# PabloAlvarado/gpitch

Measured on AMD Instinct MI355X. Metric: ELBO-steps/sec, higher is better.
Workload: dtype f64

## Files before the change

gpitch_amd/_lib.py:

```python
import ctypes as C
import os

import numpy as np

_HERE = os.path.dirname(os.path.abspath(__file__))
LIB_PATH = os.environ.get("GPITCH_AMD_LIB") or os.path.join(_HERE, "libgpitch_hip.so")

GP_OK, GP_ERR_BAD_ARG, GP_ERR_NOT_PD, GP_ERR_HIP, GP_ERR_NO_DEVICE, GP_ERR_WORKSPACE, GP_ERR_UNSUPPORTED = range(7)

(KERN_MATERN12, KERN_MATERN32, KERN_MATERN52, KERN_RBF, KERN_MERCER_MATERN12SM, KERN_MATERN12SM, KERN_MATERN32SM,
 KERN_MERCER_MATERN52SM) = range(8)
NLIN_LOGISTIC, NLIN_SOFTPLUS, NLIN_GAUSS = range(3)
(TIMER_KUF_BUILD, TIMER_COND_A, TIMER_COND_LTA, TIMER_NT_GEMM, TIMER_KUF_BAR, TIMER_CHOL, TIMER_LIK, TIMER_SMALL_GEMM,
 TIMER_HYPER, TIMER_KUF_BUILD_SM) = range(10)
TIMER_NAMES = ["kuf_build", "cond_A", "cond_LTA", "nt_gemm", "kuf_bar", "chol", "lik", "small_gemm", "hyper",
               "kuf_build_sm"]

ABI_SYMBOLS = [
    "gp_create", "gp_destroy", "gp_sync", "gp_last_error", "gp_abi_version", "gp_debug_wave_takes", "gp_debug_gemm",
    "gp_debug_hyper_contract", "gp_debug_hyper_records", "gp_debug_hyper_lean_takes", "gp_debug_cov_build", "gp_last_not_pd_index",
    "gp_kernel_build", "gp_kernel_build_f32", "gp_kernel_diag", "gp_chol_workspace_bytes", "gp_kuu_cholesky", "gp_cholesky_inplace",
    "gp_conditional_workspace_bytes", "gp_conditional_diag", "gp_conditional_diag_f32", "gp_conditional_diag_f32w", "gp_conditional_full_workspace_bytes", "gp_conditional_full", "gp_gauss_kl_workspace_bytes", "gp_gauss_kl", "gp_gauss_kl_matrix", "gp_mpd_varexp",
    "gp_mpd_predict_moments", "gp_pdgp_predict_moments", "gp_pdgp_predict_moments_reuse",
    "gp_pdgp_create", "gp_pdgp_destroy", "gp_pdgp_num_params", "gp_pdgp_layout", "gp_pdgp_workspace_bytes",
    "gp_pdgp_set_workspace", "gp_pdgp_set_precision", "gp_pdgp_set_gp_precision", "gp_pdgp_set_grad_needs", "gp_pdgp_set_overlap", "gp_pdgp_set_frames_ascending", "gp_pdgp_set_qform", "gp_pdgp_far_field", "gp_pdgp_far_field_backward", "gp_debug_pdgp_far_ranges", "gp_pdgp_set_far_act", "gp_pdgp_far_field_act", "gp_pdgp_set_scan_far", "gp_pdgp_scan_far", "gp_pdgp_set_h_far", "gp_pdgp_h_far", "gp_debug_pdgp_act_ranges", "gp_pdgp_elbo", "gp_pdgp_elbo_begin", "gp_pdgp_elbo_end", "gp_pdgp_create_subset", "gp_pdgp_cond_begin", "gp_pdgp_cond_end", "gp_pdgp_predict", "gp_pdgp_predict_reuse",
    "gp_pdgp_sample", "gp_pdgp_sample_reuse", "gp_pdgp_sample_workspace_bytes",
    "gp_overlap_merge", "gp_transform_register_logistic", "gp_transform_forward", "gp_transform_backward", "gp_poll_not_pd", "gp_check_not_pd", "gp_take_not_pd", "gp_adam_step",
    "gp_pdgp_natgrad_workspace_bytes", "gp_pdgp_natgrad_step",
    "gp_pdgp_natgrad_adaptive_workspace_bytes", "gp_pdgp_natgrad_step_adaptive", "gp_pdgp_natgrad_counts",
    "gp_sgpr_create", "gp_sgpr_destroy", "gp_sgpr_num_params", "gp_sgpr_workspace_bytes", "gp_sgpr_set_workspace", "gp_sgpr_set_precision",
    "gp_sgpr_bound", "gp_sgpr_bound_grad", "gp_sgpr_residual_grad", "gp_sgpr_exchange_doubles", "gp_sgpr_bound_begin", "gp_sgpr_bound_end", "gp_sgpr_set_graphs", "gp_sgpr_eval_counts", "gp_sgpr_predict_f", "gp_sgpr_predict_f_full", "gp_sgpr_predict_source_full", "gp_sgpr_predict_source_workspace_bytes", "gp_sgpr_predict_source", "gp_sgpr_predict_source_sparse",
    "gp_sgpr_sample_source_sparse", "gp_sgpr_sample_source_workspace_bytes",
    "gp_sgpr_predict_source_ssm", "gp_sgprb_predict_source_ssm", "gp_ssm_smooth_workspace_bytes",
    "gp_sgpr_exact_loglik_grad", "gp_sgprb_exact_loglik_grad", "gp_ssm_score_workspace_bytes",
    "gp_sgpr_sample_source_ssm", "gp_sgprb_sample_source_ssm", "gp_ssm_sample_workspace_bytes",
    "gp_sgprb_create", "gp_sgprb_destroy", "gp_sgprb_num_params", "gp_sgprb_num_windows", "gp_sgprb_workspace_bytes",
    "gp_sgprb_set_workspace", "gp_sgprb_bound_grad", "gp_sgprb_set_graphs", "gp_sgprb_eval_counts",
    "gp_sgprb_set_inducing_counts",
    "gp_sgprb_predict_f", "gp_sgprb_predict_source_workspace_bytes", "gp_sgprb_predict_source", "gp_sgprb_predict_source_sparse", "gp_sgprb_sample_source_sparse",
    "gp_timers_enable", "gp_timers_reset", "gp_timers_read",
    "gp_comm_unique_id", "gp_comm_create", "gp_comm_destroy", "gp_comm_world", "gp_comm_rank", "gp_comm_allreduce_sum",
    "gp_pdgp_elbo_pitch_sharded", "gp_pdgp_elbo_gp_sharded", "gp_sgpr_bound_grad_sharded",
    "gp_segment_gram_workspace_bytes", "gp_segment_gram", "gp_autocorr", "gp_kernfit_eval",
# ... 105 lines not shown
    if _lib is not None:
        return _lib
    import torch
    if not os.path.exists(LIB_PATH):
        raise ImportError("gpitch_amd: %s not found — build it with `python -c 'import __graft_entry__ as g; "
                          "g.build()'` (hipcc --offload-arch=gfx950); there is no CPU fallback" % LIB_PATH)
    lib = C.CDLL(LIB_PATH)
    vp, i32, i64, dbl, sz = C.c_void_p, C.c_int32, C.c_int64, C.c_double, C.c_size_t
    KD = C.POINTER(KernelDesc)
    sig = {
        "gp_create": (i32, [i32, vp, C.POINTER(vp)]),
        "gp_destroy": (i32, [vp]),
        "gp_sync": (i32, [vp]),
        "gp_last_error": (C.c_char_p, [vp]),
        "gp_abi_version": (i32, []),
        "gp_debug_wave_takes": (i32, [i32, i32, i32, i32]),
        "gp_debug_gemm": (i32, [vp, C.POINTER(DebugGemmProblem), i32, i32, i32, C.POINTER(DebugGemmFlags), i32, i32, i32, vp, sz,
                                C.POINTER(i32)]),
        "gp_debug_hyper_contract": (i32, [vp, i32, C.POINTER(DebugHyperItem), C.POINTER(DebugHyperFinish), i32,
                                          C.POINTER(DebugHyperFlags), vp, sz, C.POINTER(i32), C.POINTER(i32)]),
        "gp_debug_hyper_records": (i64, [i32, i32]),
        "gp_debug_hyper_lean_takes": (i32, [i32, i32, i32, i32, i32]),
        "gp_debug_cov_build": (i32, [vp, i32, C.POINTER(DebugCovItem), i32, vp, i32, i32, vp, sz, C.POINTER(i32), C.POINTER(i32)]),
        "gp_last_not_pd_index": (i32, [vp]),
        "gp_kernel_build": (i32, [vp, KD, vp, i32, vp, i32, vp, i64, i32]),
        "gp_kernel_build_f32": (i32, [vp, KD, vp, i32, vp, i32, vp, i64, i32]),
        "gp_kernel_diag": (i32, [vp, KD, i32, vp, i32]),
        "gp_chol_workspace_bytes": (sz, [i32]),
        "gp_kuu_cholesky": (i32, [vp, KD, vp, i32, dbl, vp, vp, vp, sz]),
        "gp_cholesky_inplace": (i32, [vp, vp, i32, i64]),
        "gp_conditional_workspace_bytes": (sz, [i32, i32]),
        "gp_conditional_diag": (i32, [vp, KD, vp, i32, vp, i32, vp, vp, i32, dbl, vp, vp, vp, sz]),
        "gp_conditional_full_workspace_bytes": (sz, [i32, i32]),
        "gp_conditional_full": (i32, [vp, KD, vp, i32, vp, i32, vp, vp, i32, dbl, vp, vp, vp, sz]),
        "gp_conditional_diag_f32": (i32, [vp, KD, vp, i32, vp, i32, vp, vp, dbl, vp, vp, vp, sz]),
        "gp_conditional_diag_f32w": (i32, [vp, KD, vp, i32, vp, i32, vp, vp, i32, dbl, vp, vp, vp, sz]),
        "gp_gauss_kl_workspace_bytes": (sz, [i32, i32]),
        "gp_gauss_kl": (i32, [vp, vp, vp, i32, KD, vp, dbl, C.POINTER(dbl), vp, sz]),
        "gp_gauss_kl_matrix": (i32, [vp, vp, vp, i32, vp, C.POINTER(dbl), vp, sz]),
        "gp_mpd_varexp": (i32, [vp, vp, vp, vp, i32, i32, i32, vp, vp, C.POINTER(dbl)]),
        "gp_mpd_predict_moments": (i32, [vp, vp, vp, vp, i32, i32, i32, vp, vp, vp, vp, vp, vp]),
        "gp_pdgp_create": (i32, [vp, C.POINTER(PdgpConfig), C.POINTER(vp)]),
        "gp_pdgp_destroy": (i32, [vp]),
        "gp_pdgp_num_params": (i64, [vp]),
        "gp_pdgp_layout": (i32, [vp, i32, C.POINTER(i64), C.POINTER(i64), C.POINTER(i64), C.POINTER(i64)]),
        "gp_pdgp_workspace_bytes": (sz, [vp]),
# ... 261 lines not shown
```

gpitch_amd/csrc/abi.hip:

```cpp
#include "engine.h"
#include "switches.h"
#include <string.h>
#include <stdlib.h>
#include <string.h>
#include <math.h>

GpTimerScope::GpTimerScope(gp_handle h_, int which_) : h(h_), which(which_) {
  if (!h || !h->timers_on) return;
  auto get = [&]() {
    hipEvent_t e;
    if (!h->event_pool.empty()) { e = h->event_pool.back(); h->event_pool.pop_back(); }
    else if (hipEventCreate(&e) != hipSuccess) e = nullptr;
    return e;
  };
  e0 = get(); e1 = get();
  if (e0) (void)hipEventRecord(e0, h->stream);
}
GpTimerScope::~GpTimerScope() {
  if (!h || !h->timers_on || !e0 || !e1) return;
  (void)hipEventRecord(e1, h->stream);
  h->pending.push_back({e0, e1, which});
}

bool gp_aux_fork(gp_handle h) {
// ... 557 lines not shown
  GP_HIP_CHECK(h, hipMemcpyAsync(host_status4, h->d_status, 4 * sizeof(int32_t), hipMemcpyDeviceToHost, h->stream));
  GP_HIP_CHECK(h, hipMemsetAsync(h->d_status, 0, 4 * sizeof(int32_t), h->stream));
  return GP_OK;
}

gp_status gp_adam_step(gp_handle h, double* fs, double* params, const double* grad, const uint8_t* tcode, double* m,
                       double* v, int64_t n, int64_t t, double lr, double beta1, double beta2, double eps) {
  if (!h) return GP_ERR_BAD_ARG;
  if (!fs || !params || !grad || !tcode || !m || !v || n < 0 || t < 1)
    return gp_fail(h, GP_ERR_BAD_ARG, "gp_adam_step: bad argument");
  return launch_adam(h, fs, params, grad, tcode, m, v, n, t, lr, beta1, beta2, eps);
}

}

const GpSwitches& gp_switches() {
  static const GpSwitches sw = []() {
    GpSwitches w;
    const char* e = getenv("GPITCH_AMD_SWITCHES");
    if (!e) return w;
    struct { const char* name; int* slot; } table[] = {
        {"strip_wave", &w.strip_wave}, {"strip_wave_f32", &w.strip_wave_f32}, {"strip_wave_roles", &w.strip_wave_roles}, {"strip_lean", &w.strip_lean},
        {"hyper_fuse", &w.hyper_fuse}, {"kufbar_split", &w.kufbar_split}, {"cond_a_early", &w.cond_a_early},
        {"blocked_256", &w.blocked_256}, {"cov_sum", &w.cov_sum}, {"hyper_sum", &w.hyper_sum}, {"chol_cluster", &w.chol_cluster}, {"aux_priority", &w.aux_priority}, {"gemm_tile32", &w.gemm_tile32}, {"nt_cover", &w.nt_cover}, {"kuf_scan", &w.kuf_scan}, {"scan_side", &w.scan_side}, {"qform", &w.qform}, {"qform_far", &w.qform_far}, {"qform_qbar", &w.qform_qbar}, {"act_far", &w.act_far}, {"scan_far", &w.scan_far}, {"h_far", &w.h_far}, {"ssm_wide", &w.ssm_wide}};
    std::string all(e);
    size_t pos = 0;
    while (pos < all.size()) {
      size_t end = all.find(',', pos);
      if (end == std::string::npos) end = all.size();
      const std::string item = all.substr(pos, end - pos);
      pos = end + 1;
      const size_t eq = item.find('=');
      if (item.empty()) continue;
      bool known = false;
      if (eq != std::string::npos)
        for (auto& t : table)
          if (item.compare(0, eq, t.name) == 0 && strlen(t.name) == eq) { *t.slot = atoi(item.c_str() + eq + 1); known = true; }
      if (!known) fprintf(stderr, "libgpitch_hip: GPITCH_AMD_SWITCHES: unknown switch '%s' ignored (gpitch_amd/csrc/switches.h)\n", item.c_str());
    }
    return w;
  }();
  return sw;
}
```

gpitch_amd/csrc/afar.hip:

```cpp
#include "engine.h"

#define AF_KAPPA (1.0 - 1.5e-12)
#define AF_SQRT3 1.7320508075688772

AfarSizes afar_sizes(int M, int N) {
  const size_t ng = ((size_t)N + AFAR_GROUP - 1) / AFAR_GROUP;
  AfarSizes s;
  s.rng = gp_align_up(ng, 32);
  s.ref = gp_align_up(2 * ng, 32);
  s.T = gp_align_up(ng * (size_t)M * 8, 32);
  s.Psi = gp_align_up(4 * (size_t)N, 32);
  s.C = gp_align_up((size_t)M * M, 32);
  return s;
}

bool afar_takes(int M, int N) {
  if (M <= 0 || N <= 0 || (M % 16) != 0 || M > 1024 || (N % AFAR_GROUP) != 0) return false;
  if ((int64_t)M * N < ((int64_t)1 << 20)) return false;
  return afar_sizes(M, N).T * 8 < ((size_t)1 << 31);
}

__global__ void __launch_bounds__(AFAR_GROUP) afar_cols_kernel(const AfarItem* __restrict__ items, const double* __restrict__ x, int N) {
  const AfarItem it = items[blockIdx.y];
  const int S = blockIdx.x, tid = threadIdx.x, n = S * AFAR_GROUP + tid, M = it.M;
// ... 60 lines not shown
        const int i = side ? M - 1 - (done + tid) : done + tid;
        const double a = side ? c * (it.z[i] - ref) : c * (ref - it.z[i]);
        const double e = exp(-a);
        ew[tid] = e; ea[tid] = e * a;
      }
      __syncthreads();
      if (act) {
        for (int r = 0; r < nn; r++) {
          const int i = side ? M - 1 - (done + r) : done + r;
          const double xv = (fac == 0 && i > j) ? 0.0 : xrow[i];
          m0 = fma(xv, ew[r], m0);
          m1 = fma(xv, ea[r], m1);
        }
      }
      done += nn;
    }
    if (act) {
      double* t = it.T + ((size_t)S * M + j) * 8 + fac * 4 + side * 2;
      t[0] = m0; t[1] = m1;
    }
  }
}

typedef double af_d4 __attribute__((ext_vector_type(4)));
typedef double af_d2 __attribute__((ext_vector_type(2)));
typedef const af_d2 __attribute__((address_space(1))) * af_gc2;
typedef af_d2 __attribute__((address_space(1))) * af_g2;

#define AF_COLS 32
#define AF_CT 2
#define AF_SB __builtin_amdgcn_sched_barrier(0)

struct AfFrag {
  af_d2 w[AF_CT][2], c[AF_CT][2];
  double tw, tc;
};

static __device__ __forceinline__ void af_mask_diag(af_d2 (&w)[2], int lc, int kq) {
#pragma unroll
  for (int h = 0; h < 2; h++) {
    const int d = 8 * h + 2 * kq - lc;
    if (d > 0) w[h].x = 0.0;
    if (d + 1 > 0) w[h].y = 0.0;
  }
}

// ... 103 lines not shown
#pragma unroll
    for (int r = 0; r < 4; r++) {
      const double v0 = aw[0][r], v1 = aw[1][r];
      *pA = af_d2{v0, v1};
      pA += 2 * ld;
      s1[0] = fma(v0, v0, s1[0]); s1[1] = fma(v1, v1, s1[1]);
      const double q = qs[16 * a + kq + 4 * r];
      dot[0] = fma(v0, q, dot[0]); dot[1] = fma(v1, q, dot[1]);
      s2[0] = fma(ac[0][r], ac[0][r], s2[0]); s2[1] = fma(ac[1][r], ac[1][r], s2[1]);
    }
  }
#pragma unroll
  for (int p = 0; p < 2; p++) {
    double t1 = 0.0, t2 = 0.0, td = 0.0;
#pragma unroll
    for (int qq = 0; qq < 4; qq++) {
      const double u1 = __shfl(s1[p], lc + 16 * qq, 64), u2 = __shfl(s2[p], lc + 16 * qq, 64), ud = __shfl(dot[p], lc + 16 * qq, 64);
      t1 = qq ? t1 + u1 : u1; t2 = qq ? t2 + u2 : u2; td = qq ? td + ud : ud;
    }
    if (kq == 0) { const int n = n0 + 2 * lc + p; it.s1[n] = t1; it.s2[n] = t2; it.dot[n] = td; }
  }
}

gp_status launch_afar(gp_handle h, const AfarItem* d_items, int count, int M, const double* x, int n) {
  if (count <= 0) return GP_OK;
  if (!afar_takes(M, n)) return gp_fail(h, GP_ERR_UNSUPPORTED, "activation far field: whole 256-frame groups, M a multiple of 16 up to 1024, strips of 2^20 entries or more");
  hipLaunchKernelGGL(afar_cols_kernel, dim3(n / AFAR_GROUP, count), dim3(AFAR_GROUP), 0, h->stream, d_items, x, n);
  hipLaunchKernelGGL(afar_t_kernel, dim3((M + 255) / 256, 4, count), dim3(256), 0, h->stream, d_items, n);
  GP_HIP_CHECK(h, hipGetLastError());
  {
    GpTimerScope ts(h, GP_TIMER_COND_A);
    hipLaunchKernelGGL(afar_prod_kernel, dim3(n / (4 * AF_COLS), count), dim3(256), 0, h->stream, d_items, n);
    GP_HIP_CHECK(h, hipGetLastError());
  }
  return GP_OK;
}
```

gpitch_amd/csrc/engine.h:

```cpp
#pragma once
#include "common.h"
#include <functional>

size_t cond_finish_item_bytes();
void cond_finish_fill(void* host_item, const double* s1, int rb1, const double* s2, int rb2, const double* dot,
                      int rbdot, DevKern k, double* fmean, double* fvar);
gp_status launch_cond_finish(gp_handle h, const void* d_items, int count, int N);
size_t kl_item_bytes();
void kl_item_fill(void* host_item, const double* q_mu, const double* q_sqrt, int M, double* out, double* g_mu,
                  double* g_sqrt);
gp_status launch_kl_white(gp_handle h, const void* d_items, int count);
size_t klu_item_bytes();
void klu_item_fill(void* host_item, const double* q_mu, const double* q_sqrt, const double* L, const double* W,
                   const double* tr_part, int nrb, int M, double* out);
gp_status launch_kl_unwhite(gp_handle h, const void* d_items, int count);
gp_status launch_elbo_finish(gp_handle h, const double* lik_partials, int nblocks, const double* kl, int nkl,
                             double* elbo, double* g_noise);
gp_status launch_mean_source(gp_handle h, const double* fmean, int P, int n, int nlin, double* out);

gp_status launch_rowdot_batched(gp_handle h, const GemmProblem* d_probs, int batch, int maxM);
gp_status launch_sub_identity_batched(gp_handle h, const GemmProblem* d_probs, int batch, int maxM);
gp_status launch_phi_batched(gp_handle h, const GemmProblem* d_probs, int batch, int maxM);
gp_status launch_rank1_tril_batched(gp_handle h, const GemmProblem* d_probs, int batch, int maxM);
gp_status launch_matvec_batched(gp_handle h, const GemmProblem* d_probs, int batch, int maxM, int trans);
// ... 57 lines not shown
  const double* A; const double* gv; const double* gm;
  const double* R; const double* alpha; const double* z;
  const double* theta;
  double* mom; double* near; double* partials;
  int64_t lda; int M, pad;
  const double* Kuf; const double* W; const int* rng; const double* T; const double* Psi;
};
int kuf_scan_nq(int ktype);
int kuf_scan_chunks(int N);
size_t kuf_scan_moment_doubles(int N, int M, int ktype);
int kuf_scan_records(int M);
gp_status launch_kuf_scan(gp_handle h, int ktype, const KufScanItem* d_items, int count, int maxM, const double* x, int n, int far = 0);

struct QfarItem {
  const double* z; const double* theta; const double* fz; const double* fx; const double* Q;
  int* rng; double* ref; double* T; double* Psi;
  int M, pad;
};
#define QFAR_GROUP 256
struct QfarSizes { size_t rng, ref, T, Psi; };
QfarSizes qfar_sizes(int M, int N, int m);
bool qfar_takes(int M, int N, int m);
gp_status launch_qfar_tables(gp_handle h, const QfarItem* d_items, int count, int M, int m, const double* x, int n);

struct QbarItem {
  const double* Kuf; int64_t ldk; const double* gv; const double* gm;
  const double* z; const double* theta; const double* fz;
  const int* rng; const double* ref; const double* Psi;
  int* rng2; int* tS;
  double* CnF; double* CFF; double* cn; double* cF;
  double* Um; double* Vp; double* Wv;
  double* Qbar; double* v;
  int M, pad;
};
#define QBAR_MAX_TILES 64
#define QBAR_MAX_NF 64
struct QbarSizes { size_t rng2, tS, CnF, CFF, cn, cF, Um, Wv; };
QbarSizes qbar_sizes(int M, int N, int m);
bool qbar_takes(int M, int N, int m);
gp_status launch_qbar(gp_handle h, const QbarItem* d_items, int count, int M, int m, int n);

struct AfarItem {
  const double* z; const double* theta; const double* W; const double* C; const double* Kuf; const double* q_mu;
  double* A; double* s1; double* s2; double* dot;
  int* rng; double* ref; double* T; double* Psi;
  int64_t ld; int M, pad;
};
#define AFAR_GROUP 256
struct AfarSizes { size_t rng, ref, T, Psi, C; };
AfarSizes afar_sizes(int M, int N);
bool afar_takes(int M, int N);
gp_status launch_afar(gp_handle h, const AfarItem* d_items, int count, int M, const double* x, int n);

struct HfarItem {
  const double* A; const double* Kuf; const double* W; const double* gv; const double* gm;
  const int* rng; const double* T; const double* Psi;
  double* Yn; double* Yf; double* up; int* flag;
  double* slabs; double* upart;
  int64_t ld; int M, gp;
};
struct HfarSizes { size_t Yn, Yf, up, flag; };
HfarSizes hfar_sizes(int M, int N);
bool hfar_takes(int M, int N);
gp_status launch_hfar(gp_handle h, const HfarItem* d_items, int count, int M, int n, int nsplit, int charges);

#define CB_NB 128
#define CB_MAX_PANELS 8

struct CondDescLayout {
  size_t chol_ptrs, w_ptrs, Ms, lds, f1, f1u, f2, finish;
  size_t fq, finish_q;
  size_t cov_uu, cov_uf, feat_zuu, feat_zuf, feat_x;
  size_t blk_mats[CB_MAX_PANELS], blk_w[CB_MAX_PANELS], blk_M[CB_MAX_PANELS], blk_gemm[CB_MAX_PANELS][4];
  size_t diag_mats, diag_w, diag_M, diag_ld;
  size_t bytes;
// ... 57 lines not shown
```

gpitch_amd/csrc/pdgp_bwd.hip:

```cpp
#include "pdgp_plan.h"
#include <string.h>
#include <stdlib.h>

enum BwdSlot { S_H = 0, S_U, S_HLQ, S_QW_MU, S_QW_L, S_GQ_MU, S_GQ_L,
               S_E, S_CHAIN, S_R = S_CHAIN + CH_R, S_ALPHA = S_CHAIN + CH_ALPHA, S_G = S_CHAIN + CH_G, S_WB_R1 = S_CHAIN + CH_COUNT, S_WB_L,
               S_QE, S_QR, S_QALPHA, S_QQ, S_QT, S_QHH, S_QU,
               S_AC,
               S_COUNT };
static_assert(S_COUNT <= PDGP_KLTR_SLOT, "pdgp_plan.h: the backward slots must stay below the KL trace slot");
static inline const GemmProblem* slot_probs(gp_pdgp_plan p, int slot) { return (const GemmProblem*)(p->d_misc + p->off.bwd[slot]); }
static inline GemmProblem& host_prob(gp_pdgp_plan p, int slot, int i, int M) {
  GemmProblem& r = *((GemmProblem*)(p->h_misc.data() + p->off.bwd[slot]) + i);
  gemm_problem_square(r, M);
  return r;
}

void pdgp_upload_qform(gp_pdgp_plan p, const double* params) {
  for (int i = 0; i < p->routes.nq; i++) {
    const int g = p->routes.q0 + i;
    const PdgpGP& q = p->gps[g];
    const CondTask& t = p->cb.tasks[g];
    const BwdBufs& b = p->bw[g];
    const int M = q.M;
    auto P = [&](int slot) -> GemmProblem& { return host_prob(p, slot, i, M); };
// ... 7 lines not shown
      const size_t nfz = gp_align_up((size_t)2 * sm_mpad(q.m) * M, 32);
      it = QfarItem{t.z, t.kern.theta, t.feat, t.feat + nfz, b.Q, b.qf_rng, b.qf_ref, b.qf_T, b.qf_Psi, M, 0};
    }
  }
}

__global__ void __launch_bounds__(256) qform_guard_kernel(const GemmProblem* __restrict__ probs, int g0, double cmax, int32_t* status) {
  const GemmProblem p = probs[blockIdx.x];
  const double* L = p.v0;
  const double* W = p.B;
  double sl = 0.0, sw = 0.0;
  for (int idx = threadIdx.x; idx < p.M * p.M; idx += 256)
    if (idx % p.M <= idx / p.M) { sl = fma(L[idx], L[idx], sl); sw = fma(W[idx], W[idx], sw); }
  __shared__ double red[2][4];
  for (int o = 32; o > 0; o >>= 1) { sl += __shfl_down(sl, o, 64); sw += __shfl_down(sw, o, 64); }
  if ((threadIdx.x & 63) == 0) { red[0][threadIdx.x >> 6] = sl; red[1][threadIdx.x >> 6] = sw; }
  __syncthreads();
  if (threadIdx.x == 0) {
    const double c = ((red[0][0] + red[0][1]) + (red[0][2] + red[0][3])) * ((red[1][0] + red[1][1]) + (red[1][2] + red[1][3]));
    if (!(c <= cmax * (double)p.M * (double)p.M)) { status[0] = 4; status[1] = 0; status[2] = g0 + (int)blockIdx.x; }
  }
}

gp_status pdgp_qform_join(gp_pdgp_plan p);
static gp_status qform_chain(gp_pdgp_plan p, const double* x, int n, bool far_wait, hipEvent_t tables_done = nullptr) {
  gp_handle h = p->h;
  const int nq = p->routes.nq, maxM = p->maxM;
  GP_CHECK(launch_chain_e(h, slot_probs(p, S_QE), nq, maxM));
  GP_CHECK(launch_chain_r_alpha(h, slot_probs(p, S_QR), slot_probs(p, S_QALPHA), nq, maxM));
  GemmFlags f; f.triB = TRI_LOWER;
  GP_CHECK(launch_gemm_batched(h, slot_probs(p, S_QQ), nq, maxM, maxM, f));
  if (p->routes.q_far) {
    if (far_wait && hipStreamWaitEvent(h->stream, h->ev_feat, 0) != hipSuccess) return gp_fail(h, GP_ERR_HIP, "event hand-over to the helper stream failed");
    GP_CHECK(launch_qfar_tables(h, (const QfarItem*)(p->d_misc + p->off.qf_items), nq, maxM, p->gps[p->routes.q0].m, x, n));
  }
  if (tables_done && hipEventRecord(tables_done, h->stream) != hipSuccess) return gp_fail(h, GP_ERR_HIP, "event hand-over from the helper stream failed");
  hipLaunchKernelGGL(qform_guard_kernel, dim3(nq), dim3(256), 0, h->stream, slot_probs(p, S_QQ), p->routes.q0, (double)GP_QFORM_COND_MAX, h->d_status);
  if (hipGetLastError() != hipSuccess) return gp_fail(h, GP_ERR_HIP, "qform guard launch failed");
  return GP_OK;
}

gp_status pdgp_qform_prepare(gp_pdgp_plan p, const double* x, int n) {
  gp_handle h = p->h;
  h->guard_pending = false;
  if (p->routes.nq <= 0) return GP_OK;
  bool aux = (n >= 4096) && p->overlap >= 2 && h->aux_stream && !h->aux_active;
  if (aux && p->routes.q_far && !p->cb.feat_ready) aux = false;
  if (aux && !h->ev_q && hipEventCreateWithFlags(&h->ev_q, hipEventDisableTiming) != hipSuccess) { h->ev_q = nullptr; aux = false; }
  if (aux && !h->ev_guard && hipEventCreateWithFlags(&h->ev_guard, hipEventDisableTiming) != hipSuccess) { h->ev_guard = nullptr; aux = false; }
  gp_status st;
  { GpStreamScope on(h, aux ? h->aux_stream : nullptr); st = qform_chain(p, x, n, aux, aux ? h->ev_q : nullptr); }
  hipError_t e = hipSuccess;
  if (aux) {
    e = hipEventRecord(h->ev_guard, h->aux_stream);
    if (e == hipSuccess) h->guard_pending = true;
    if (e == hipSuccess && st == GP_OK) e = hipStreamWaitEvent(h->stream, h->ev_q, 0);
    if (st != GP_OK) (void)pdgp_qform_join(p);
  }
  GP_CHECK(st);
  if (e != hipSuccess) return gp_fail(h, GP_ERR_HIP, "event hand-over from the helper stream failed");
// ... 554 lines not shown
```

gpitch_amd/csrc/qfar.hip:

```cpp
#include "engine.h"
#include "cov_entry.h"

QfarSizes qfar_sizes(int M, int N, int m) {
  const size_t ng = ((size_t)N + QFAR_GROUP - 1) / QFAR_GROUP, nf = 2 * (size_t)sm_mpad(m);
  QfarSizes s;
  s.rng = gp_align_up(ng, 32);
  s.ref = gp_align_up(2 * ng, 32);
  s.T = gp_align_up(ng * (size_t)M * 2 * nf, 32);
  s.Psi = gp_align_up(2 * nf * (size_t)N, 32);
  return s;
}

bool qfar_takes(int M, int N, int m) {
  if (M <= 0 || N <= 0 || m < 1 || m > 32 || (M % 64) != 0 || M > 1024 || (N % QFAR_GROUP) != 0) return false;
  const QfarSizes s = qfar_sizes(M, N, m);
  return s.T * 8 < ((size_t)1 << 31) && s.Psi * 8 < ((size_t)1 << 31);
}

__global__ void __launch_bounds__(QFAR_GROUP) qfar_cols_kernel(const QfarItem* __restrict__ items, const double* __restrict__ x,
                                                               int N, int nf) {
  const QfarItem it = items[blockIdx.y];
  const int S = blockIdx.x, tid = threadIdx.x, n = S * QFAR_GROUP + tid, M = it.M;
  const double var = it.theta[0], ls = it.theta[1];
  const double b = x[n] / ls;
// ... 78 lines not shown
    for (int r = done + tid; r < cend; r += 256) {
      int lo = 0, hi = nc - 1;
      while (lo < hi) { const int mid = (lo + hi) >> 1; if (cnt[mid] > r) hi = mid; else lo = mid + 1; }
      const double a = it.z[row_of(r)] / ls, bref = sref[lo];
      ew[r] = exp(side ? -(a - bref) : -(bref - a));
    }
    __syncthreads();
    for (int q = 0; q < nc; q++) {
      if (c0 + q > 0) t *= dec[q];
      const int k1 = cnt[q];
      while (done < k1) {
#pragma unroll
        for (int r = 0; r < 16; r++) t = fma(qn[r], ew[done + r] * fn[r], t);
        done += 16;
        if (done < M) fetch(done);
      }
      const int S = side ? ng - 1 - (c0 + q) : c0 + q;
      if (act) it.T[((size_t)S * M + j) * (2 * nf) + side * nf + f] = t;
    }
    bcarry = sref[nc - 1];
  }
}

gp_status launch_qfar_tables(gp_handle h, const QfarItem* d_items, int count, int M, int m, const double* x, int n) {
  if (count <= 0) return GP_OK;
  if (!qfar_takes(M, n, m)) return gp_fail(h, GP_ERR_UNSUPPORTED, "far-field tables: whole 256-frame groups, M a multiple of 64 up to 1024");
  const int nf = 2 * sm_mpad(m);
  hipLaunchKernelGGL(qfar_cols_kernel, dim3(n / QFAR_GROUP, count), dim3(QFAR_GROUP), 0, h->stream, d_items, x, n, nf);
  hipLaunchKernelGGL(qfar_t_kernel, dim3((M * nf + 255) / 256, 2, count), dim3(256), 0, h->stream, d_items, n, nf);
  GP_HIP_CHECK(h, hipGetLastError());
  return GP_OK;
}
```

gpitch_amd/csrc/switches.h:

```cpp
#pragma once
struct GpSwitches {
  int strip_wave = 1, strip_wave_f32 = (1 << 1) | (1 << 2) | (1 << 3) | (1 << 5), strip_wave_roles = (1 << 1) | (1 << 2) | (1 << 3) | (1 << 5), strip_lean = 1, hyper_fuse = 1, kufbar_split = -1,
      cond_a_early = 1, blocked_256 = 1, cov_sum = 1, hyper_sum = 1, chol_cluster = 1, aux_priority = 1, gemm_tile32 = 320, nt_cover = 0, kuf_scan = 1, scan_side = 1, qform = 1, qform_far = 1, qform_qbar = 1, act_far = 1, scan_far = 1, h_far = 1, ssm_wide = 0;
};
#define GP_QFORM_COND_MAX 4.0
const GpSwitches& gp_switches();
```

include/gpitch_abi.h:

```cpp
#ifndef GPITCH_ABI_H
#define GPITCH_ABI_H

#include <stddef.h>
#include <stdint.h>

#ifdef __cplusplus
extern "C" {
#endif

#define GPITCH_ABI_VERSION 1

typedef int32_t gp_status;
enum {
  GP_OK = 0,
  GP_ERR_BAD_ARG = 1,
  GP_ERR_NOT_PD = 2,
  GP_ERR_HIP = 3,
  GP_ERR_NO_DEVICE = 4,
  GP_ERR_WORKSPACE = 5,
  GP_ERR_UNSUPPORTED = 6
};

enum {
  GP_KERN_MATERN12 = 0,
// ... 58 lines not shown
  const double* p_uf; const double* p_uu; const double* gv_sum; double* g_theta;
  const double* gz_uf; const double* gz_uu; double* g_z;
  int32_t np_uf, np_uu, cb_uf, cb_uu, n1, pad_;
} gp_debug_hyper_finish;
typedef struct {
  int32_t with_gz, use_mfma, g32_items, lean_items, gscale_items, n2_shared;
  const double* x2_shared;
} gp_debug_hyper_flags;
gp_status gp_debug_hyper_contract(gp_handle h, int32_t entry, const gp_debug_hyper_item* items, const gp_debug_hyper_finish* fins,
                                  int32_t count, const gp_debug_hyper_flags* flags, void* workspace, size_t workspace_bytes,
                                  int32_t* nparts, int32_t* taken);
int64_t gp_debug_hyper_records(int32_t N, int32_t M);
int32_t gp_debug_hyper_lean_takes(int32_t type, int32_t m, int32_t n1, int32_t n2, int32_t count);
typedef struct {
  gp_kernel_desc kern;
  const double* x1; const double* x2;
  void* out; double* feat;
  int64_t ld; double diag_add;
  int32_t n1, n2, accumulate, f32out;
} gp_debug_cov_item;
gp_status gp_debug_cov_build(gp_handle h, int32_t entry, const gp_debug_cov_item* items, int32_t count,
                             const double* x2_shared, int32_t n2_shared, int32_t engine_strips,
                             void* workspace, size_t workspace_bytes, int32_t* form, int32_t* row_seg);
int32_t gp_last_not_pd_index(gp_handle h);

gp_status gp_kernel_build(gp_handle h, const gp_kernel_desc* kern, const double* x1, int32_t n1,
                          const double* x2, int32_t n2, double* out, int64_t ld, int32_t accumulate);
gp_status gp_kernel_build_f32(gp_handle h, const gp_kernel_desc* kern, const double* x1, int32_t n1,
                              const double* x2, int32_t n2, float* out, int64_t ld, int32_t accumulate);
gp_status gp_kernel_diag(gp_handle h, const gp_kernel_desc* kern, int32_t n, double* out, int32_t accumulate);

size_t gp_chol_workspace_bytes(int32_t M);
gp_status gp_kuu_cholesky(gp_handle h, const gp_kernel_desc* kern, const double* z, int32_t M, double jitter,
                          double* L, double* Linv, void* workspace, size_t workspace_bytes);
gp_status gp_cholesky_inplace(gp_handle h, double* A, int32_t M, int64_t ld);

size_t gp_conditional_workspace_bytes(int32_t N, int32_t M);
gp_status gp_conditional_diag(gp_handle h, const gp_kernel_desc* kern, const double* xnew, int32_t N,
                              const double* z, int32_t M, const double* q_mu, const double* q_sqrt,
                              int32_t whiten, double jitter, double* fmean, double* fvar,
                              void* workspace, size_t workspace_bytes);

gp_status gp_conditional_diag_f32(gp_handle h, const gp_kernel_desc* kern, const double* xnew, int32_t N,
                                  const double* z, int32_t M, const double* q_mu, const double* q_sqrt,
                                  double jitter, double* fmean, double* fvar,
                                  void* workspace, size_t workspace_bytes);
// ... 339 lines not shown
```

Before: 120.9.

## Add LDS-tiled far-field table kernels and a row-blocked qform guard

Adds new versions of the activation and Q-route far-field table kernels. They stage 16-row tiles of the W/C or Q matrices and the z features in shared memory with double buffering and prefetch, and precompute per-row exponential weights per chunk. This is meant to replace strided, uncoalesced global reads in the original table scans. The qform guard also moves to a 1024-thread, row-blocked, vectorised norm reduction. All of this sits behind a new far_tables switch that is on by default, and a debug entry point is added to test the kernels in isolation. The price is more shared memory and synchronisation per block and fewer threads in the activation tables kernel.

```diff
diff --git a/gpitch_amd/_lib.py b/gpitch_amd/_lib.py
--- a/gpitch_amd/_lib.py
+++ b/gpitch_amd/_lib.py
@@ -18,7 +18,7 @@
 
 ABI_SYMBOLS = [
     "gp_create", "gp_destroy", "gp_sync", "gp_last_error", "gp_abi_version", "gp_debug_wave_takes", "gp_debug_gemm",
-    "gp_debug_hyper_contract", "gp_debug_hyper_records", "gp_debug_hyper_lean_takes", "gp_debug_cov_build", "gp_last_not_pd_index",
+    "gp_debug_hyper_contract", "gp_debug_hyper_records", "gp_debug_hyper_lean_takes", "gp_debug_cov_build", "gp_debug_far_tables", "gp_last_not_pd_index",
     "gp_kernel_build", "gp_kernel_build_f32", "gp_kernel_diag", "gp_chol_workspace_bytes", "gp_kuu_cholesky", "gp_cholesky_inplace",
     "gp_conditional_workspace_bytes", "gp_conditional_diag", "gp_conditional_diag_f32", "gp_conditional_diag_f32w", "gp_conditional_full_workspace_bytes", "gp_conditional_full", "gp_gauss_kl_workspace_bytes", "gp_gauss_kl", "gp_gauss_kl_matrix", "gp_mpd_varexp",
     "gp_mpd_predict_moments", "gp_pdgp_predict_moments", "gp_pdgp_predict_moments_reuse",
@@ -170,6 +170,7 @@
         "gp_debug_hyper_records": (i64, [i32, i32]),
         "gp_debug_hyper_lean_takes": (i32, [i32, i32, i32, i32, i32]),
         "gp_debug_cov_build": (i32, [vp, i32, C.POINTER(DebugCovItem), i32, vp, i32, i32, vp, sz, C.POINTER(i32), C.POINTER(i32)]),
+        "gp_debug_far_tables": (i32, [vp, i32, i32, vp, vp, vp, vp, vp, vp, vp, vp, i32, i32, i32, vp, sz]),
         "gp_last_not_pd_index": (i32, [vp]),
         "gp_kernel_build": (i32, [vp, KD, vp, i32, vp, i32, vp, i64, i32]),
         "gp_kernel_build_f32": (i32, [vp, KD, vp, i32, vp, i32, vp, i64, i32]),
diff --git a/gpitch_amd/csrc/abi.hip b/gpitch_amd/csrc/abi.hip
--- a/gpitch_amd/csrc/abi.hip
+++ b/gpitch_amd/csrc/abi.hip
@@ -603,7 +603,7 @@
     struct { const char* name; int* slot; } table[] = {
         {"strip_wave", &w.strip_wave}, {"strip_wave_f32", &w.strip_wave_f32}, {"strip_wave_roles", &w.strip_wave_roles}, {"strip_lean", &w.strip_lean},
         {"hyper_fuse", &w.hyper_fuse}, {"kufbar_split", &w.kufbar_split}, {"cond_a_early", &w.cond_a_early},
-        {"blocked_256", &w.blocked_256}, {"cov_sum", &w.cov_sum}, {"hyper_sum", &w.hyper_sum}, {"chol_cluster", &w.chol_cluster}, {"aux_priority", &w.aux_priority}, {"gemm_tile32", &w.gemm_tile32}, {"nt_cover", &w.nt_cover}, {"kuf_scan", &w.kuf_scan}, {"scan_side", &w.scan_side}, {"qform", &w.qform}, {"qform_far", &w.qform_far}, {"qform_qbar", &w.qform_qbar}, {"act_far", &w.act_far}, {"scan_far", &w.scan_far}, {"h_far", &w.h_far}, {"ssm_wide", &w.ssm_wide}};
+        {"blocked_256", &w.blocked_256}, {"cov_sum", &w.cov_sum}, {"hyper_sum", &w.hyper_sum}, {"chol_cluster", &w.chol_cluster}, {"aux_priority", &w.aux_priority}, {"gemm_tile32", &w.gemm_tile32}, {"nt_cover", &w.nt_cover}, {"kuf_scan", &w.kuf_scan}, {"scan_side", &w.scan_side}, {"qform", &w.qform}, {"qform_far", &w.qform_far}, {"qform_qbar", &w.qform_qbar}, {"act_far", &w.act_far}, {"scan_far", &w.scan_far}, {"h_far", &w.h_far}, {"far_tables", &w.far_tables}, {"ssm_wide", &w.ssm_wide}};
     std::string all(e);
     size_t pos = 0;
     while (pos < all.size()) {
diff --git a/gpitch_amd/csrc/afar.hip b/gpitch_amd/csrc/afar.hip
--- a/gpitch_amd/csrc/afar.hip
+++ b/gpitch_amd/csrc/afar.hip
@@ -106,6 +106,113 @@
   }
 }
 
+typedef double aft_d2 __attribute__((ext_vector_type(2)));
+#define AFT_ROWS 64
+#define AFT_CHUNK 64
+#define AFT_LD 17
+__global__ void __launch_bounds__(AFT_ROWS) afar_t_tiled_kernel(const AfarItem* __restrict__ items, int N) {
+  const AfarItem it = items[blockIdx.z];
+  const int side = blockIdx.y & 1, fac = blockIdx.y >> 1, tid = threadIdx.x, M = it.M, ng = N / AFAR_GROUP;
+  const int j0 = blockIdx.x * AFT_ROWS, j = j0 + tid;
+  const bool act = j < M;
+  const double c = AF_SQRT3 / it.theta[1];
+  const double* __restrict__ X = fac ? it.C : it.W;
+  __shared__ int cnt[AFT_CHUNK];
+  __shared__ double sref[AFT_CHUNK], sa[AFT_CHUNK], se[AFT_CHUNK];
+  __shared__ double ew[1024], ea[1024];
+  __shared__ double xs[2][AFT_ROWS * AFT_LD];
+  const int nt = M / 16;
+  auto tile_i0 = [&](int t) { return side ? M - 16 * (t + 1) : 16 * t; };
+  aft_d2 xn[8];
+  auto request = [&](int t) {
+    const int i0 = tile_i0(t);
+#pragma unroll
+    for (int k = 0; k < 8; k++) {
+      const int row = min(j0 + 8 * k + (tid >> 3), M - 1);
+      xn[k] = *(const aft_d2*)(X + (size_t)row * M + i0 + 2 * (tid & 7));
+    }
+  };
+  auto deposit = [&](int t) {
+    double* b = xs[t & 1];
+#pragma unroll
+    for (int k = 0; k < 8; k++) {
+      double* d = b + (8 * k + (tid >> 3)) * AFT_LD + 2 * (tid & 7);
+      d[0] = xn[k].x; d[1] = xn[k].y;
+    }
+  };
+  request(0);
+  deposit(0);
+  if (nt > 1) request(1);
+  __syncthreads();
+  int have = 0;
+  double m0 = 0.0, m1 = 0.0, rcarry = 0.0;
+  int done = 0;
+  for (int c0 = 0; c0 < ng; c0 += AFT_CHUNK) {
+    const int nc = min(AFT_CHUNK, ng - c0);
+    __syncthreads();
+    if (tid < nc) {
+      const int S = side ? ng - 1 - (c0 + tid) : c0 + tid;
+      cnt[tid] = side ? M - it.rng[2 * S + 1] : it.rng[2 * S];
+      sref[tid] = it.ref[2 * S + side];
+    }
+    __syncthreads();
+    int mine = done;
+    double a = 0.0, e = 1.0;
+    if (tid < nc) {
+      for (int q = 0; q <= tid; q++) mine = max(mine, cnt[q]);
+      const double refprev = tid > 0 ? sref[tid - 1] : rcarry, ref = sref[tid];
+      a = side ? c * (refprev - ref) : c * (ref - refprev);
+      e = exp(-a);
+    }
+    __syncthreads();
+    if (tid < nc) { cnt[tid] = mine; sa[tid] = a; se[tid] = e; }
+    __syncthreads();
+    const int cend = min(cnt[nc - 1], M);
+    for (int r = done + tid; r < cend; r += AFT_ROWS) {
+      int lo = 0, hi = nc - 1;
+      while (lo < hi) { const int mid = (lo + hi) >> 1; if (cnt[mid] > r) hi = mid; else lo = mid + 1; }
+      const int i = side ? M - 1 - r : r;
+      const double ref = sref[lo];
+      const double ai = side ? c * (it.z[i] - ref) : c * (ref - it.z[i]);
+      const double ei = exp(-ai);
+      ew[r] = ei; ea[r] = ei * ai;
+    }
+    __syncthreads();
+    for (int q = 0; q < nc; q++) {
+      if (c0 + q > 0) {
+        const double aq = sa[q], eq = se[q];
+        m1 = eq * fma(aq, m0, m1);
+        m0 = eq * m0;
+      }
+      const int k1 = min(cnt[q], M);
+      while (done < k1) {
+        const int t = done >> 4, r1 = min(k1, 16 * (t + 1));
+        if (t != have) {
+          deposit(t);
+          if (t + 1 < nt) request(t + 1);
+          __syncthreads();
+          have = t;
+        }
+        const double* xr = xs[t & 1] + tid * AFT_LD;
+        for (int r = done; r < r1; r++) {
+          const int q16 = r & 15, i = side ? M - 1 - r : r;
+          const double xl = xr[side ? 15 - q16 : q16];
+          const double xv = (fac == 0 && i > j) ? 0.0 : xl;
+          m0 = fma(xv, ew[r], m0);
+          m1 = fma(xv, ea[r], m1);
+        }
+        done = r1;
+      }
+      if (act) {
+        const int S = side ? ng - 1 - (c0 + q) : c0 + q;
+        double* t = it.T + ((size_t)S * M + j) * 8 + fac * 4 + side * 2;
+        t[0] = m0; t[1] = m1;
+      }
+    }
+    rcarry = sref[nc - 1];
+  }
+}
+
 typedef double af_d4 __attribute__((ext_vector_type(4)));
 typedef double af_d2 __attribute__((ext_vector_type(2)));
 typedef const af_d2 __attribute__((address_space(1))) * af_gc2;
@@ -255,11 +362,16 @@
   }
 }
 
+void launch_afar_t(gp_handle h, const AfarItem* d_items, int count, int M, int n, bool tiled) {
+  if (tiled) hipLaunchKernelGGL(afar_t_tiled_kernel, dim3((M + AFT_ROWS - 1) / AFT_ROWS, 4, count), dim3(AFT_ROWS), 0, h->stream, d_items, n);
+  else hipLaunchKernelGGL(afar_t_kernel, dim3((M + 255) / 256, 4, count), dim3(256), 0, h->stream, d_items, n);
+}
+
 gp_status launch_afar(gp_handle h, const AfarItem* d_items, int count, int M, const double* x, int n) {
   if (count <= 0) return GP_OK;
   if (!afar_takes(M, n)) return gp_fail(h, GP_ERR_UNSUPPORTED, "activation far field: whole 256-frame groups, M a multiple of 16 up to 1024, strips of 2^20 entries or more");
   hipLaunchKernelGGL(afar_cols_kernel, dim3(n / AFAR_GROUP, count), dim3(AFAR_GROUP), 0, h->stream, d_items, x, n);
-  hipLaunchKernelGGL(afar_t_kernel, dim3((M + 255) / 256, 4, count), dim3(256), 0, h->stream, d_items, n);
+  launch_afar_t(h, d_items, count, M, n, gp_switches().far_tables != 0);
   GP_HIP_CHECK(h, hipGetLastError());
   {
     GpTimerScope ts(h, GP_TIMER_COND_A);
diff --git a/gpitch_amd/csrc/engine.h b/gpitch_amd/csrc/engine.h
--- a/gpitch_amd/csrc/engine.h
+++ b/gpitch_amd/csrc/engine.h
@@ -103,6 +103,7 @@
 QfarSizes qfar_sizes(int M, int N, int m);
 bool qfar_takes(int M, int N, int m);
 gp_status launch_qfar_tables(gp_handle h, const QfarItem* d_items, int count, int M, int m, const double* x, int n);
+void launch_qfar_t(gp_handle h, const QfarItem* d_items, int count, int M, int nf, int n, bool lds);
 
 struct QbarItem {
   const double* Kuf; int64_t ldk; const double* gv; const double* gm;
@@ -132,6 +133,7 @@
 AfarSizes afar_sizes(int M, int N);
 bool afar_takes(int M, int N);
 gp_status launch_afar(gp_handle h, const AfarItem* d_items, int count, int M, const double* x, int n);
+void launch_afar_t(gp_handle h, const AfarItem* d_items, int count, int M, int n, bool tiled);
 
 struct HfarItem {
   const double* A; const double* Kuf; const double* W; const double* gv; const double* gm;
diff --git a/gpitch_amd/csrc/far_debug.hip b/gpitch_amd/csrc/far_debug.hip
--- /dev/null
+++ b/gpitch_amd/csrc/far_debug.hip
@@ -0,0 +1,36 @@
+#include "engine.h"
+#include <string.h>
+
+static_assert(sizeof(AfarItem) <= 256 && sizeof(QfarItem) <= 256, "gp_debug_far_tables: include/gpitch_abi.h promises 256 bytes of workspace");
+
+static bool fd_al16(const void* p) { return (((uintptr_t)p) & 15) == 0; }
+
+extern "C" gp_status gp_debug_far_tables(gp_handle h, int32_t which, int32_t form, const double* X, const double* X2, const double* z,
+                                         const double* theta, const double* fz, int32_t* rng, double* ref, double* T, int32_t M,
+                                         int32_t N, int32_t nf, void* workspace, size_t workspace_bytes) {
+  if (!h) return GP_ERR_BAD_ARG;
+  if (which < 0 || which > 1 || form < 0 || form > 1 || !X || !z || !theta || !rng || !ref || !T || M <= 0 || M > 1024 || N <= 0 ||
+      !fd_al16(X))
+    return gp_fail(h, GP_ERR_BAD_ARG, "gp_debug_far_tables: bad argument");
+  if (!workspace || !fd_al16(workspace) || workspace_bytes < 256)
+    return gp_fail(h, GP_ERR_WORKSPACE, "gp_debug_far_tables: workspace too small or not 16-byte aligned");
+  if (which == 0) {
+    if (!X2 || !fd_al16(X2) || fz || nf != 0 || (M % 16) != 0 || (N % AFAR_GROUP) != 0)
+      return gp_fail(h, GP_ERR_BAD_ARG, "gp_debug_far_tables: the activations' tables take W and C, M a multiple of 16, whole 256-frame groups");
+    AfarItem it;
+    memset(&it, 0, sizeof(it));
+    it.z = z; it.theta = theta; it.W = X; it.C = X2; it.rng = rng; it.ref = ref; it.T = T; it.M = M;
+    GP_HIP_CHECK(h, hipMemcpyAsync(workspace, &it, sizeof(it), hipMemcpyHostToDevice, h->stream));
+    launch_afar_t(h, (const AfarItem*)workspace, 1, M, N, form != 0);
+  } else {
+    if (X2 || !fz || !fd_al16(fz) || nf <= 0 || nf > 64 || (nf % 8) != 0 || (M % 64) != 0 || (N % QFAR_GROUP) != 0)
+      return gp_fail(h, GP_ERR_BAD_ARG, "gp_debug_far_tables: the Q route's tables take Q and the z features, M a multiple of 64, nf of 8, whole 256-frame groups");
+    QfarItem it;
+    memset(&it, 0, sizeof(it));
+    it.z = z; it.theta = theta; it.fz = fz; it.Q = X; it.rng = rng; it.ref = ref; it.T = T; it.M = M;
+    GP_HIP_CHECK(h, hipMemcpyAsync(workspace, &it, sizeof(it), hipMemcpyHostToDevice, h->stream));
+    launch_qfar_t(h, (const QfarItem*)workspace, 1, M, nf, N, form != 0);
+  }
+  GP_HIP_CHECK(h, hipGetLastError());
+  return GP_OK;
+}
diff --git a/gpitch_amd/csrc/pdgp_bwd.hip b/gpitch_amd/csrc/pdgp_bwd.hip
--- a/gpitch_amd/csrc/pdgp_bwd.hip
+++ b/gpitch_amd/csrc/pdgp_bwd.hip
@@ -53,6 +53,49 @@
   }
 }
 
+typedef double qg_d2 __attribute__((ext_vector_type(2)));
+__global__ void __launch_bounds__(1024) qform_guard_rows_kernel(const GemmProblem* __restrict__ probs, int g0, double cmax, int32_t* status) {
+  const GemmProblem p = probs[blockIdx.x];
+  const double* L = p.v0;
+  const double* W = p.B;
+  const int M = p.M, lane = threadIdx.x & 63, wave = threadIdx.x >> 6;
+  const bool wide = (M & 1) == 0 && ((((uintptr_t)L) | ((uintptr_t)W)) & 15) == 0;
+  double sl[4] = {0.0, 0.0, 0.0, 0.0}, sw[4] = {0.0, 0.0, 0.0, 0.0};
+  for (int rb = wave; rb < M; rb += 64) {
+    const int rtop = min(rb + 48, M - 1);
+    for (int k = lane; 2 * k <= rtop; k += 64) {
+      qg_d2 l[4], w[4];
+#pragma unroll
+      for (int u = 0; u < 4; u++) {
+        const int r = rb + 16 * u;
+        l[u] = w[u] = qg_d2{0.0, 0.0};
+        if (r < M && 2 * k <= r) {
+          const size_t o = (size_t)r * M + 2 * k;
+          if (wide) { l[u] = *(const qg_d2*)(L + o); w[u] = *(const qg_d2*)(W + o); }
+          else { l[u].x = L[o]; w[u].x = W[o]; if (2 * k + 1 <= r) { l[u].y = L[o + 1]; w[u].y = W[o + 1]; } }
+          if (2 * k + 1 > r) { l[u].y = 0.0; w[u].y = 0.0; }
+        }
+      }
+#pragma unroll
+      for (int u = 0; u < 4; u++) {
+        sl[u] = fma(l[u].x, l[u].x, sl[u]); sl[u] = fma(l[u].y, l[u].y, sl[u]);
+        sw[u] = fma(w[u].x, w[u].x, sw[u]); sw[u] = fma(w[u].y, w[u].y, sw[u]);
+      }
+    }
+  }
+  double tl = (sl[0] + sl[1]) + (sl[2] + sl[3]), tw = (sw[0] + sw[1]) + (sw[2] + sw[3]);
+  __shared__ double red[2][16];
+  for (int o = 32; o > 0; o >>= 1) { tl += __shfl_down(tl, o, 64); tw += __shfl_down(tw, o, 64); }
+  if (lane == 0) { red[0][wave] = tl; red[1][wave] = tw; }
+  __syncthreads();
+  if (threadIdx.x == 0) {
+    double al = red[0][0], aw = red[1][0];
+    for (int q = 1; q < 16; q++) { al += red[0][q]; aw += red[1][q]; }
+    const double c = al * aw;
+    if (!(c <= cmax * (double)M * (double)M)) { status[0] = 4; status[1] = 0; status[2] = g0 + (int)blockIdx.x; }
+  }
+}
+
 gp_status pdgp_qform_join(gp_pdgp_plan p);
 static gp_status qform_chain(gp_pdgp_plan p, const double* x, int n, bool far_wait, hipEvent_t tables_done = nullptr) {
   gp_handle h = p->h;
@@ -66,7 +109,10 @@
     GP_CHECK(launch_qfar_tables(h, (const QfarItem*)(p->d_misc + p->off.qf_items), nq, maxM, p->gps[p->routes.q0].m, x, n));
   }
   if (tables_done && hipEventRecord(tables_done, h->stream) != hipSuccess) return gp_fail(h, GP_ERR_HIP, "event hand-over from the helper stream failed");
-  hipLaunchKernelGGL(qform_guard_kernel, dim3(nq), dim3(256), 0, h->stream, slot_probs(p, S_QQ), p->routes.q0, (double)GP_QFORM_COND_MAX, h->d_status);
+  if (gp_switches().far_tables != 0)
+    hipLaunchKernelGGL(qform_guard_rows_kernel, dim3(nq), dim3(1024), 0, h->stream, slot_probs(p, S_QQ), p->routes.q0, (double)GP_QFORM_COND_MAX, h->d_status);
+  else
+    hipLaunchKernelGGL(qform_guard_kernel, dim3(nq), dim3(256), 0, h->stream, slot_probs(p, S_QQ), p->routes.q0, (double)GP_QFORM_COND_MAX, h->d_status);
   if (hipGetLastError() != hipSuccess) return gp_fail(h, GP_ERR_HIP, "qform guard launch failed");
   return GP_OK;
 }
diff --git a/gpitch_amd/csrc/qfar.hip b/gpitch_amd/csrc/qfar.hip
--- a/gpitch_amd/csrc/qfar.hip
+++ b/gpitch_amd/csrc/qfar.hip
@@ -124,12 +124,118 @@
   }
 }
 
+#define QFL_ROWS 32
+#define QFL_LDP 65
+#define QFL_LD 33
+typedef double qfl_d2 __attribute__((ext_vector_type(2)));
+template <int QFL_EPT>
+__global__ void __launch_bounds__(256, 4) qfar_t_lds_kernel(const QfarItem* __restrict__ items, int N, int nf) {
+  const QfarItem it = items[blockIdx.z];
+  const int side = blockIdx.y, tid = threadIdx.x, M = it.M, ng = N / QFAR_GROUP;
+  const int j0 = blockIdx.x * QFL_ROWS, npr = nf / 16 + ((nf & 15) ? 1 : 0);
+  const double ls = it.theta[1];
+  __shared__ int cnt[QFT_CHUNK];
+  __shared__ double sref[QFT_CHUNK], dec[QFT_CHUNK];
+  __shared__ double ew[1024];
+  __shared__ double qs[2][16 * QFL_LD], ps[2][16 * QFL_LDP];
+  auto row_of = [&](int r) { return side ? M - 16 * (r / 16 + 1) + (r % 16) : r; };
+  const int jl = tid >> 3, fg = tid & 7;
+  qfl_d2 qn;
+  double fn[4];
+  auto request = [&](int done) {
+    const int i0 = row_of(done);
+    qn = *(const qfl_d2*)(it.Q + (size_t)(j0 + (tid >> 3)) * M + i0 + 2 * (tid & 7));
+#pragma unroll
+    for (int k = 0; k < 4; k++) {
+      const int f = (tid >> 4) + 16 * k;
+      fn[k] = (k < npr && f < nf) ? it.fz[(size_t)f * M + i0 + (tid & 15)] : 0.0;
+    }
+  };
+  auto deposit = [&](int done) {
+    const int b = (done >> 4) & 1;
+    qs[b][(2 * (tid & 7)) * QFL_LD + (tid >> 3)] = qn.x;
+    qs[b][(2 * (tid & 7) + 1) * QFL_LD + (tid >> 3)] = qn.y;
+    const double w = ew[done + (tid & 15)];
+#pragma unroll
+    for (int k = 0; k < 4; k++) {
+      const int f = (tid >> 4) + 16 * k;
+      if (k < npr && f < nf) ps[b][(tid & 15) * QFL_LDP + f] = w * fn[k];
+    }
+  };
+  double t[QFL_EPT];
+#pragma unroll
+  for (int k = 0; k < QFL_EPT; k++) t[k] = 0.0;
+  double bcarry = 0.0;
+  int done = 0;
+  request(0);
+  for (int c0 = 0; c0 < ng; c0 += QFT_CHUNK) {
+    const int nc = min(QFT_CHUNK, ng - c0);
+    __syncthreads();
+    if (tid < nc) {
+      const int S = side ? ng - 1 - (c0 + tid) : c0 + tid;
+      cnt[tid] = side ? M - it.rng[2 * S + 1] : it.rng[2 * S];
+      sref[tid] = it.ref[2 * S + side];
+    }
+    __syncthreads();
+    int mine = done;
+    double d = 1.0;
+    if (tid < nc) {
+      for (int q = 0; q <= tid; q++) mine = max(mine, cnt[q]);
+      const double bprev = tid > 0 ? sref[tid - 1] : bcarry, bref = sref[tid];
+      d = exp(side ? -(bprev - bref) : -(bref - bprev));
+    }
+    __syncthreads();
+    if (tid < nc) { cnt[tid] = mine; dec[tid] = d; }
+    __syncthreads();
+    const int cend = cnt[nc - 1];
+    for (int r = done + tid; r < cend; r += 256) {
+      int lo = 0, hi = nc - 1;
+      while (lo < hi) { const int mid = (lo + hi) >> 1; if (cnt[mid] > r) hi = mid; else lo = mid + 1; }
+      const double a = it.z[row_of(r)] / ls, bref = sref[lo];
+      ew[r] = exp(side ? -(a - bref) : -(bref - a));
+    }
+    __syncthreads();
+    for (int q = 0; q < nc; q++) {
+      if (c0 + q > 0) {
+        const double dq = dec[q];
+#pragma unroll
+        for (int k = 0; k < QFL_EPT; k++) t[k] *= dq;
+      }
+      const int k1 = cnt[q];
+      while (done < k1) {
+        deposit(done);
+        if (done + 16 < M) request(done + 16);
+        __syncthreads();
+        const double* qb = qs[(done >> 4) & 1];
+        const double* pb = ps[(done >> 4) & 1];
+#pragma unroll
+        for (int r = 0; r < 16; r++) {
+          const double qv = qb[r * QFL_LD + jl];
+#pragma unroll
+          for (int k = 0; k < QFL_EPT; k++) t[k] = fma(qv, pb[r * QFL_LDP + fg + 8 * k], t[k]);
+        }
+        done += 16;
+      }
+      const int S = side ? ng - 1 - (c0 + q) : c0 + q;
+#pragma unroll
+      for (int k = 0; k < QFL_EPT; k++) it.T[((size_t)S * M + j0 + jl) * (2 * nf) + side * nf + fg + 8 * k] = t[k];
+    }
+    bcarry = sref[nc - 1];
+  }
+}
+
+void launch_qfar_t(gp_handle h, const QfarItem* d_items, int count, int M, int nf, int n, bool lds) {
+#define QFL_CASE(E) case E: hipLaunchKernelGGL(qfar_t_lds_kernel<E>, dim3(M / QFL_ROWS, 2, count), dim3(256), 0, h->stream, d_items, n, nf); break;
+  if (lds) switch (nf / 8) { QFL_CASE(1) QFL_CASE(2) QFL_CASE(3) QFL_CASE(4) QFL_CASE(5) QFL_CASE(6) QFL_CASE(7) QFL_CASE(8) }
+  else hipLaunchKernelGGL(qfar_t_kernel, dim3((M * nf + 255) / 256, 2, count), dim3(256), 0, h->stream, d_items, n, nf);
+}
+
 gp_status launch_qfar_tables(gp_handle h, const QfarItem* d_items, int count, int M, int m, const double* x, int n) {
   if (count <= 0) return GP_OK;
   if (!qfar_takes(M, n, m)) return gp_fail(h, GP_ERR_UNSUPPORTED, "far-field tables: whole 256-frame groups, M a multiple of 64 up to 1024");
   const int nf = 2 * sm_mpad(m);
   hipLaunchKernelGGL(qfar_cols_kernel, dim3(n / QFAR_GROUP, count), dim3(QFAR_GROUP), 0, h->stream, d_items, x, n, nf);
-  hipLaunchKernelGGL(qfar_t_kernel, dim3((M * nf + 255) / 256, 2, count), dim3(256), 0, h->stream, d_items, n, nf);
+  launch_qfar_t(h, d_items, count, M, nf, n, gp_switches().far_tables != 0);
   GP_HIP_CHECK(h, hipGetLastError());
   return GP_OK;
 }
diff --git a/gpitch_amd/csrc/switches.h b/gpitch_amd/csrc/switches.h
--- a/gpitch_amd/csrc/switches.h
+++ b/gpitch_amd/csrc/switches.h
@@ -1,7 +1,7 @@
 #pragma once
 struct GpSwitches {
   int strip_wave = 1, strip_wave_f32 = (1 << 1) | (1 << 2) | (1 << 3) | (1 << 5), strip_wave_roles = (1 << 1) | (1 << 2) | (1 << 3) | (1 << 5), strip_lean = 1, hyper_fuse = 1, kufbar_split = -1,
-      cond_a_early = 1, blocked_256 = 1, cov_sum = 1, hyper_sum = 1, chol_cluster = 1, aux_priority = 1, gemm_tile32 = 320, nt_cover = 0, kuf_scan = 1, scan_side = 1, qform = 1, qform_far = 1, qform_qbar = 1, act_far = 1, scan_far = 1, h_far = 1, ssm_wide = 0;
+      cond_a_early = 1, blocked_256 = 1, cov_sum = 1, hyper_sum = 1, chol_cluster = 1, aux_priority = 1, gemm_tile32 = 320, nt_cover = 0, kuf_scan = 1, scan_side = 1, qform = 1, qform_far = 1, qform_qbar = 1, act_far = 1, scan_far = 1, h_far = 1, far_tables = 1, ssm_wide = 0;
 };
 #define GP_QFORM_COND_MAX 4.0
 const GpSwitches& gp_switches();
diff --git a/include/gpitch_abi.h b/include/gpitch_abi.h
--- a/include/gpitch_abi.h
+++ b/include/gpitch_abi.h
@@ -104,6 +104,9 @@
 gp_status gp_debug_cov_build(gp_handle h, int32_t entry, const gp_debug_cov_item* items, int32_t count,
                              const double* x2_shared, int32_t n2_shared, int32_t engine_strips,
                              void* workspace, size_t workspace_bytes, int32_t* form, int32_t* row_seg);
+gp_status gp_debug_far_tables(gp_handle h, int32_t which, int32_t form, const double* X, const double* X2, const double* z,
+                              const double* theta, const double* fz, int32_t* rng, double* ref, double* T, int32_t M, int32_t N,
+                              int32_t nf, void* workspace, size_t workspace_bytes);
 int32_t gp_last_not_pd_index(gp_handle h);
 
 gp_status gp_kernel_build(gp_handle h, const gp_kernel_desc* kern, const double* x1, int32_t n1,
```

Result: faster. 128.3, median of 6 (+6.1%).
